# 0xMiden/miden-vm

Hardware: NVIDIA H100
Metric: trace cells/sec proved (higher is better)
Workload: dtype u64

## Files before the change

miden-vm_b200/csrc/kernels.cu:

```cuda
#include "kernels.cuh"
#include "poseidon2.cuh"
#include "poseidon2_fast2.cuh"
#include "ntt2.cuh"
#include "blake3.cuh"
#include "keccak.cuh"
#include "rescue.cuh"
#include <algorithm>
#include <cstdio>

namespace mk {

static unsigned long long g_launches = 0;
unsigned long long launch_count() { return g_launches; }
void count_launch() { ++g_launches; }
void reset_launch_count() { g_launches = 0; }
#define COUNT_LAUNCH() (++g_launches)

void upload_constants() {
    cudaMemcpyToSymbol(p2::D_RC_EXT_INITIAL, p2::P2_RC_EXT_INITIAL, sizeof(u64) * 48);
    cudaMemcpyToSymbol(p2::D_RC_INTERNAL, p2::P2_RC_INTERNAL, sizeof(u64) * 22);
    cudaMemcpyToSymbol(p2::D_RC_EXT_TERMINAL, p2::P2_RC_EXT_TERMINAL, sizeof(u64) * 48);
    cudaMemcpyToSymbol(rsc::D_ARK1, rsc::RESCUE_ARK1, sizeof(u64) * 84);
    cudaMemcpyToSymbol(rsc::D_ARK2, rsc::RESCUE_ARK2, sizeof(u64) * 84);
}

#ifdef MDN_EMULATED
static inline void st_release_sys(u64* p, u64 v) { __atomic_store_n(p, v, __ATOMIC_RELEASE); }
static inline u64 ld_acquire_sys(const u64* p) { return __atomic_load_n(p, __ATOMIC_ACQUIRE); }
static constexpr long long BARRIER_TIMEOUT = 600ll * 1000000000ll;
#else
__device__ __forceinline__ void st_release_sys(u64* p, u64 v) { asm volatile("st.release.sys.global.u64 [%0], %1;" ::"l"(p), "l"(v) : "memory"); }
__device__ __forceinline__ u64 ld_acquire_sys(const u64* p) { u64 v; asm volatile("ld.acquire.sys.global.u64 %0, [%1];" : "=l"(v) : "l"(p) : "memory"); return v; }
static constexpr long long BARRIER_TIMEOUT = 30000000000ll;
#endif
__device__ __forceinline__ void push_u2(const PushDst& d, size_t idx, size_t owner_key, ulonglong2 v) {
    if (d.mode == PUSH_ALL) {
        for (u32 g = 0; g < d.world; g++) reinterpret_cast<ulonglong2*>(d.pp.p[g])[idx] = v;
    } else {
        u32 g = d.mode == PUSH_OWNER ? (u32)(owner_key >> d.owner_shift) : d.rank;
        reinterpret_cast<ulonglong2*>(d.pp.p[g])[idx] = v;
    }
}
struct BarrierArgs { PeerPtrs flags; u32 rank, world; u64 epoch; u32* err; };
__global__ void k_barrier(BarrierArgs a) {
    u32 p = threadIdx.x;
    if (p < a.world) { __threadfence_system(); st_release_sys(a.flags.p[p] + a.rank, a.epoch); }
    __syncthreads();
    if (p < a.world) {
        long long t0 = clock64();
        while (ld_acquire_sys(a.flags.p[a.rank] + p) < a.epoch) {
            if (clock64() - t0 > BARRIER_TIMEOUT) { atomicOr(a.err, 8u); break; }
#ifdef MDN_EMULATED
            emu::cpu_relax();
#endif
        }
    }
}
void launch_barrier(const PeerPtrs& flags, u32 rank, u32 world, u64 epoch, u32* err, cudaStream_t st) {
    BarrierArgs a; a.flags = flags; a.rank = rank; a.world = world; a.epoch = epoch; a.err = err;
    k_barrier<<<1, 32, 0, st>>>(a);
    COUNT_LAUNCH();
}
struct PushArgs { const u64* src; PeerPtrs dst; u32 rank, world; size_t n; };
__global__ void __launch_bounds__(256) k_push(PushArgs a) {
    size_t stride = (size_t)gridDim.x * blockDim.x, i0 = (size_t)blockIdx.x * blockDim.x + threadIdx.x;
    if ((a.n & 1) == 0 && (((size_t)a.src) & 15) == 0) {
        const ulonglong2* s2 = reinterpret_cast<const ulonglong2*>(a.src);
        for (size_t i = i0; i < a.n / 2; i += stride) {
            ulonglong2 v = s2[i];
            for (u32 g = 0; g < a.world; g++) if (g != a.rank) reinterpret_cast<ulonglong2*>(a.dst.p[g])[i] = v;
        }
    } else {
        for (size_t i = i0; i < a.n; i += stride) {
            u64 v = a.src[i];
            for (u32 g = 0; g < a.world; g++) if (g != a.rank) a.dst.p[g][i] = v;
        }
    }
}
void launch_push(const u64* src, const PeerPtrs& dst, u32 rank, u32 world, size_t n, cudaStream_t st) {
    if (!n || world <= 1) return;
    PushArgs a; a.src = src; a.dst = dst; a.rank = rank; a.world = world; a.n = n;
    unsigned blocks = (unsigned)std::min<size_t>((n / 2 + 255) / 256 + 1, 132 * 8);
    k_push<<<blocks, 256, 0, st>>>(a);
    COUNT_LAUNCH();
}

struct TransposeDst { PeerPtrs dst; PeerPtrs bad; u32 world; };
__global__ void k_transpose(const u64* __restrict__ src, TransposeDst d, u32 n_rows, u32 width, size_t col_stride, u32 row0) {
    __shared__ u64 tile[32][33];
    u32 r0 = blockIdx.x * 32, c0 = blockIdx.y * 32;
    bool any_bad = false;
    for (u32 i = threadIdx.y; i < 32; i += 8) {
        u32 r = r0 + i, c = c0 + threadIdx.x;
        if (r < n_rows && c < width) {
            u64 v = src[(size_t)r * width + c];
            any_bad |= (v >= gl::P);
            tile[i][threadIdx.x] = v;
        }
    }
    if (any_bad) for (u32 g = 0; g < d.world; g++) if (d.bad.p[g]) atomicOr(reinterpret_cast<u32*>(d.bad.p[g]), 1u);
    __syncthreads();
    for (u32 i = threadIdx.y; i < 32; i += 8) {
        u32 c = c0 + i, r = r0 + threadIdx.x;
        if (r < n_rows && c < width) {
            u64 v = tile[threadIdx.x][i];
            size_t o = (size_t)c * col_stride + row0 + r;
            for (u32 g = 0; g < d.world; g++) d.dst.p[g][o] = v;
        }
    }
}
void launch_transpose_rm_to_cm(const u64* src, u64* dst, u32 n_rows, u32 width, u32* d_bad_flag, cudaStream_t st) {
    TransposeDst d{}; d.dst.p[0] = dst; d.bad.p[0] = reinterpret_cast<u64*>(d_bad_flag); d.world = 1;
    dim3 grid((n_rows + 31) / 32, (width + 31) / 32), block(32, 8);
    k_transpose<<<grid, block, 0, st>>>(src, d, n_rows, width, (size_t)n_rows, 0u);
    COUNT_LAUNCH();
}
void launch_transpose_slice_push(const u64* src_slice, const PeerPtrs& dst_cm, const PeerPtrs& bad, u32 world, u32 row0, u32 n_rows_slice,
                                 u32 n_rows_total, u32 width, cudaStream_t st) {
    if (!n_rows_slice || !width) return;
    TransposeDst d{}; d.dst = dst_cm; d.bad = bad; d.world = world;
    dim3 grid((n_rows_slice + 31) / 32, (width + 31) / 32), block(32, 8);
    k_transpose<<<grid, block, 0, st>>>(src_slice, d, n_rows_slice, width, (size_t)n_rows_total, row0);
    COUNT_LAUNCH();
}

static constexpr int NTT_THREADS = 256;
static inline unsigned ntt_threads(u32 m, u32 log_cols) {
    u32 g = (m + log_cols >= 3) ? (1u << (m + log_cols - 3)) : 1u;
    if (g < 32) g = 32;
    if (g > 256) g = 256;
    return g;
}

__device__ __forceinline__ u64 w_pow(const u64* __restrict__ hi, const u64* __restrict__ lo, u32 lo_bits, u64 e) {
    return gl::mul(hi[e >> lo_bits], lo[e & ((1ull << lo_bits) - 1)]);
}

#define NTT_BOUNDS __launch_bounds__(NTT_THREADS)
template <int N1C, int N2C>
__global__ void NTT_BOUNDS k_intt_strided(u64* cols, size_t col_stride, NttTables T, u32 log_c) {
    extern __shared__ u64 sm[];
    ntt2::intt_strided_block<N1C, N2C>(blockIdx.x, blockIdx.y, sm, cols, col_stride, T, log_c);
}
template <int N2C>
__global__ void NTT_BOUNDS k_intt_contig(u64* cols, size_t col_stride, NttTables T) {
    extern __shared__ u64 sm[];
    ntt2::intt_contig_block<N2C>(blockIdx.x, blockIdx.y, sm, cols, col_stride, T);
}
template <int N1C, int N2C>
__global__ void NTT_BOUNDS k_fwd_contig(const FwdItem* __restrict__ items, NttTables T, PremulTables Pm) {
    extern __shared__ u64 sm[];
    ntt2::fwd_contig_block<N1C, N2C>(blockIdx.x, blockIdx.y, sm, items, T, Pm);
}
template <int N1C, int N2C>
__global__ void NTT_BOUNDS k_fwd_strided(const FwdItem* __restrict__ items, NttTables T, u32 log_c) {
    extern __shared__ u64 sm[];
    ntt2::fwd_strided_block<N1C, N2C>(blockIdx.x, blockIdx.y, sm, items, T, log_c);
}
#define NTT_SPECIALISED(X) X(8, 8) X(8, 9) X(9, 9) X(9, 10) X(10, 10) X(10, 11) X(11, 11)

template <int N1C, int N2C>
static void launch_intt_t(u64* cols, size_t col_stride, u32 n_cols, const NttTables& T, u32 log_c, cudaStream_t st) {
    u32 N1 = 1u << T.n1, N2 = 1u << T.n2, C = 1u << log_c;
    if (T.n1 > 0) {
        size_t smem = ntt2::smem_words_strided(T.n1, log_c) * sizeof(u64);
        cudaFuncSetAttribute(k_intt_strided<N1C, N2C>, cudaFuncAttributeMaxDynamicSharedMemorySize, (int)smem);
        k_intt_strided<N1C, N2C><<<dim3(N2 / C, n_cols), ntt_threads(T.n1, log_c), smem, st>>>(cols, col_stride, T, log_c);
        COUNT_LAUNCH();
    }
    size_t smem = ntt2::smem_words_contig_inv(T.n2) * sizeof(u64);
    k_intt_contig<N2C><<<dim3(N1, n_cols), ntt_threads(T.n2, 0), smem, st>>>(cols, col_stride, T);
    COUNT_LAUNCH();
}
void launch_intt(u64* cols, size_t col_stride, u32 n_cols, const NttTables& T, cudaStream_t st) {
    u32 log_c = T.n1 >= 12 ? 0 : 12 - T.n1; if (log_c > T.n2) log_c = T.n2;
#define X(a, b) if (T.n1 == a && T.n2 == b) { launch_intt_t<a, b>(cols, col_stride, n_cols, T, log_c, st); return; }
    NTT_SPECIALISED(X)
#undef X
    launch_intt_t<-1, -1>(cols, col_stride, n_cols, T, log_c, st);
}
template <int N1C, int N2C>
static void launch_fwd_t(const FwdItem* d_items, u32 n_items, const NttTables& T, const PremulTables& Pm, u32 log_c, cudaStream_t st) {
    u32 N1 = 1u << T.n1, N2 = 1u << T.n2, C = 1u << log_c;
    size_t smem = ntt2::smem_words_contig_fwd(T.n2) * sizeof(u64);
    k_fwd_contig<N1C, N2C><<<dim3(N1, n_items), ntt_threads(T.n2, 0), smem, st>>>(d_items, T, Pm);
    COUNT_LAUNCH();
    if (T.n1 > 0) {
        size_t smem2 = ntt2::smem_words_strided(T.n1, log_c) * sizeof(u64);
        cudaFuncSetAttribute(k_fwd_strided<N1C, N2C>, cudaFuncAttributeMaxDynamicSharedMemorySize, (int)smem2);
        k_fwd_strided<N1C, N2C><<<dim3(N2 / C, n_items), ntt_threads(T.n1, log_c), smem2, st>>>(d_items, T, log_c);
        COUNT_LAUNCH();
    }
}
void launch_fwd_ntt(const FwdItem* d_items, u32 n_items, const NttTables& T, const PremulTables& Pm, cudaStream_t st) {
    u32 log_c = T.n1 >= 12 ? 0 : 12 - T.n1; if (log_c > T.n2) log_c = T.n2;
#define X(a, b) if (T.n1 == a && T.n2 == b) { launch_fwd_t<a, b>(d_items, n_items, T, Pm, log_c, st); return; }
    NTT_SPECIALISED(X)
#undef X
    launch_fwd_t<-1, -1>(d_items, n_items, T, Pm, log_c, st);
}

static constexpr int HASH_THREADS = 128;
static constexpr int HASH_MIN_BLOCKS = 6;

enum { PERM_P2 = 0, PERM_RPO = 3, PERM_RPX = 4 };
template <int PERM>
__device__ __forceinline__ void alg_permute(u64* s) {
    if constexpr (PERM == PERM_RPO) rsc::rpo_permute(s);
    else if constexpr (PERM == PERM_RPX) rsc::rpx_permute(s);
    else p2f::permute(s);
}
#define ALG_BOUNDS(PERM) __launch_bounds__(HASH_THREADS, (PERM) == PERM_P2 ? HASH_MIN_BLOCKS : 1)
#define ALG_DISPATCH(perm, CALL) do { if ((perm) == PERM_RPO) { CALL(PERM_RPO); } else if ((perm) == PERM_RPX) { CALL(PERM_RPX); } else { CALL(PERM_P2); } } while (0)

template <int PERM>
__global__ void ALG_BOUNDS(PERM) k_leaf_hash(LeafArgs a, u32 log_n, u32 log_b, const u64* __restrict__ prev,
                                                            u32 prev_log_n, u64* __restrict__ states_out,
                                                            PushDst dig, u32 has_dig, u32 t0, u32 nt) {
    size_t L = (size_t)1 << (log_n + log_b);
    size_t idx = (size_t)blockIdx.x * blockDim.x + threadIdx.x;
    if (idx >= ((size_t)nt << log_n)) return;
    u32 t = t0 + (u32)(idx >> log_n);
    u32 r = (u32)(idx & (((size_t)1 << log_n) - 1));
    size_t pos = ((size_t)t << log_n) + r;
    u64 s[12];
    if (prev) {
        size_t Lp = (size_t)1 << (prev_log_n + log_b);
        size_t pp = ((size_t)t << prev_log_n) + (r & ((1u << prev_log_n) - 1));
#pragma unroll
        for (int k = 0; k < 12; k++) s[k] = prev[k * Lp + pp];
    } else {
#pragma unroll
        for (int k = 0; k < 12; k++) s[k] = 0;
    }
    for (int m = 0; m < a.n_mats; m++) {
        const u64* base = a.m[m].base + pos;
        u32 w = a.m[m].width;
        for (u32 c0 = 0; c0 < w; c0 += 8) {
#pragma unroll
            for (u32 k = 0; k < 8; k++) s[k] = (c0 + k < w) ? base[(size_t)(c0 + k) * L] : 0ull;
            alg_permute<PERM>(s);
        }
    }
    if (states_out) {
#pragma unroll
        for (int k = 0; k < 12; k++) states_out[k * L + pos] = glf::canon(s[k]);
    }
    if (has_dig) {
        size_t i = ((size_t)r << log_b) | t;
        push_u2(dig, 2 * i, i, make_ulonglong2(glf::canon(s[0]), glf::canon(s[1])));
        push_u2(dig, 2 * i + 1, i, make_ulonglong2(glf::canon(s[2]), glf::canon(s[3])));
    }
}
template <int PERM>
static void launch_leaf_hash_t(const LeafArgs& a, u32 log_n, u32 log_blowup, const u64* prev_states, u32 prev_log_n,
                               u64* states_out, const PushDst* dig, u32 t0, u32 nt, cudaStream_t st) {
    size_t cnt = (size_t)nt << log_n;
    unsigned blocks = (unsigned)((cnt + HASH_THREADS - 1) / HASH_THREADS);
    PushDst d = dig ? *dig : local_dst(nullptr);
    k_leaf_hash<PERM><<<blocks, HASH_THREADS, 0, st>>>(a, log_n, log_blowup, prev_states, prev_log_n, states_out, d, dig ? 1u : 0u, t0, nt);
    COUNT_LAUNCH();
}
void launch_leaf_hash(const LeafArgs& a, u32 log_n, u32 log_blowup, const u64* prev_states, u32 prev_log_n,
                      u64* states_out, const PushDst* dig, u32 t0, u32 nt, cudaStream_t st, int perm) {
#define X(PM) launch_leaf_hash_t<PM>(a, log_n, log_blowup, prev_states, prev_log_n, states_out, dig, t0, nt, st)
    ALG_DISPATCH(perm, X);
#undef X
}

template <int PERM>
__global__ void ALG_BOUNDS(PERM) k_compress(const u64* __restrict__ ch, u64* __restrict__ par, size_t n) {
    size_t i = (size_t)blockIdx.x * blockDim.x + threadIdx.x;
    if (i >= n) return;
    const ulonglong2* c = reinterpret_cast<const ulonglong2*>(ch + i * 8);
    ulonglong2 a0 = c[0], a1 = c[1], b0 = c[2], b1 = c[3];
    u64 s[12] = {a0.x, a0.y, a1.x, a1.y, b0.x, b0.y, b1.x, b1.y, 0, 0, 0, 0};
    alg_permute<PERM>(s);
    ulonglong2* d = reinterpret_cast<ulonglong2*>(par + i * 4);
    d[0] = make_ulonglong2(glf::canon(s[0]), glf::canon(s[1]));
    d[1] = make_ulonglong2(glf::canon(s[2]), glf::canon(s[3]));
}
template <int PERM>
static void launch_compress_layer_t(const u64* children, u64* parents, size_t n_parents, cudaStream_t st) {
    unsigned blocks = (unsigned)((n_parents + HASH_THREADS - 1) / HASH_THREADS);
    k_compress<PERM><<<blocks, HASH_THREADS, 0, st>>>(children, parents, n_parents);
    COUNT_LAUNCH();
}
void launch_compress_layer(const u64* children, u64* parents, size_t n_parents, cudaStream_t st, int perm) {
#define X(PM) launch_compress_layer_t<PM>(children, parents, n_parents, st)
    ALG_DISPATCH(perm, X);
#undef X
}

template <int PERM>
__global__ void __launch_bounds__(HASH_THREADS) k_fri_leaf(const u64* __restrict__ ev, size_t q, u32 la, PushDst dig, u32 log_b, u32 t0, u32 log_nt) {
    size_t idx = (size_t)blockIdx.x * blockDim.x + threadIdx.x;
    if (idx >= ((q >> log_b) << log_nt)) return;
    size_t i = ((idx >> log_nt) << log_b) | (t0 + (idx & ((1u << log_nt) - 1)));
    const ulonglong2* e = reinterpret_cast<const ulonglong2*>(ev);
    u64 s[12];
#pragma unroll
    for (int k = 0; k < 12; k++) s[k] = 0;
    u32 a = 1u << la;
    for (u32 j0 = 0; j0 < a; j0 += 4) {
#pragma unroll
        for (u32 j = 0; j < 4; j++) {
            if (j0 + j < a) {
                ulonglong2 v = e[i + (size_t)gl::bitrev32(j0 + j, la) * q];
                s[2 * j] = v.x; s[2 * j + 1] = v.y;
            } else { s[2 * j] = 0; s[2 * j + 1] = 0; }
        }
        alg_permute<PERM>(s);
    }
    push_u2(dig, 2 * i, i, make_ulonglong2(glf::canon(s[0]), glf::canon(s[1])));
    push_u2(dig, 2 * i + 1, i, make_ulonglong2(glf::canon(s[2]), glf::canon(s[3])));
}
static inline u32 log2_exact(u32 v) { u32 l = 0; while ((1u << l) < v) l++; return l; }
template <int PERM>
static void launch_fri_leaf_hash_t(const u64* evals, size_t rows, u32 log_arity, const PushDst& digests, u32 log_b, u32 t0, u32 nt, cudaStream_t st) {
    if (rows < ((size_t)1 << log_b)) { log_b = 0; t0 = 0; nt = 1; }
    size_t cnt = (rows >> log_b) * nt;
    unsigned blocks = (unsigned)((cnt + HASH_THREADS - 1) / HASH_THREADS);
    k_fri_leaf<PERM><<<blocks, HASH_THREADS, 0, st>>>(evals, rows, log_arity, digests, log_b, t0, log2_exact(nt));
    COUNT_LAUNCH();
}
void launch_fri_leaf_hash(const u64* evals, size_t rows, u32 log_arity, const PushDst& digests, u32 log_b, u32 t0, u32 nt, cudaStream_t st, int perm) {
#define X(PM) launch_fri_leaf_hash_t<PM>(evals, rows, log_arity, digests, log_b, t0, nt, st)
    ALG_DISPATCH(perm, X);
#undef X
}

__global__ void k_p2_batch(u64* st, size_t n) {
    size_t i = (size_t)blockIdx.x * blockDim.x + threadIdx.x;
    if (i >= n) return;
    u64 s[12];
#pragma unroll
    for (int k = 0; k < 12; k++) s[k] = st[i * 12 + k];
    p2f::permute(s);
#pragma unroll
    for (int k = 0; k < 12; k++) st[i * 12 + k] = glf::canon(s[k]);
}
void launch_poseidon2_batch(u64* states, size_t n, cudaStream_t st) {
    k_p2_batch<<<(unsigned)((n + 127) / 128), 128, 0, st>>>(states, n);
// ... 782 lines not shown
```

miden-vm_b200/csrc/ntt2.cuh:

```cuda
#pragma once
#include "poseidon2_fast2.cuh"
#include "kernels.cuh"
#include "tma.cuh"

namespace ntt2 {
using gl::u64;
using gl::u32;

#if defined(__CUDA_ARCH__) || defined(MDN_EMULATED)
#define NTT2_FOR(i, n) for (u32 i = threadIdx.x; i < (u32)(n); i += blockDim.x)
#define NTT2_SYNC() __syncthreads()
#else
#define NTT2_FOR(i, n) for (u32 i = 0; i < (u32)(n); i++)
#define NTT2_SYNC() ((void)0)
#endif

GL_HD u32 tile_off(u32 idx, u32 cc, u32 log_cols) {
    u32 o = (idx << log_cols) + cc;
    return log_cols ? o : o + (o >> 3);
}
GL_HD u32 tile_words(u32 m, u32 log_cols) {
    u32 n = 1u << (m + log_cols);
    return log_cols ? n : n + (n >> 3) + 1;
}
GL_HD u32 tw_off(u32 m, u32 log_cols) { return (tile_words(m, log_cols) + 1u) & ~1u; }
GL_HD size_t smem_words_contig_fwd(u32 n2) { return (size_t)tw_off(n2, 0) + ((size_t)1 << n2) + 2; }
GL_HD size_t smem_words_contig_inv(u32 n2) { return (size_t)tw_off(n2, 0) + ((size_t)1 << n2) / 2 + 4; }
GL_HD size_t smem_words_strided(u32 n1, u32 log_c) { return (size_t)tw_off(n1, log_c) + ((size_t)1 << n1) / 2 + 4; }

GL_HD void load_chunk(u64* x, const u64* src, u32 n) {
#if defined(__CUDA_ARCH__)
    if (n >= 2 && (((size_t)src) & 15) == 0) {
        const ulonglong2* s2 = reinterpret_cast<const ulonglong2*>(src);
        NTT2_FOR(i, n / 2) { ulonglong2 v = s2[i]; x[tile_off(2 * i, 0, 0)] = v.x; x[tile_off(2 * i + 1, 0, 0)] = v.y; }
        return;
    }
#endif
    NTT2_FOR(i, n) x[tile_off(i, 0, 0)] = src[i];
}
GL_HD void store_chunk_canon(u64* dst, const u64* x, u32 n) {
#if defined(__CUDA_ARCH__)
    if (n >= 2 && (((size_t)dst) & 15) == 0) {
        ulonglong2* d2 = reinterpret_cast<ulonglong2*>(dst);
        NTT2_FOR(i, n / 2) d2[i] = make_ulonglong2(glf::canon_cc(x[tile_off(2 * i, 0, 0)]), glf::canon_cc(x[tile_off(2 * i + 1, 0, 0)]));
        return;
    }
#endif
    NTT2_FOR(i, n) dst[i] = glf::canon_cc(x[tile_off(i, 0, 0)]);
}

struct TableLoad { bool async; };
GL_HD TableLoad table_load(u64* dst, const u64* src, u32 words, u64* bar) {
#if defined(__CUDA_ARCH__)
    const u32 bytes = (words * 8u + 15u) & ~15u;
    if (words >= 64 && ((((size_t)src) | ((size_t)dst)) & 15) == 0) {
        if (threadIdx.x == 0) { tma::mbar_init(bar, 1); }
        __syncthreads();
        if (threadIdx.x == 0) { tma::expect_tx(bar, bytes); tma::bulk_g2s(dst, src, bytes, bar); }
        return TableLoad{true};
    }
#endif
    (void)bar;
    NTT2_FOR(i, words) dst[i] = src[i];
    return TableLoad{false};
}
GL_HD void table_wait(TableLoad t, u64* bar) {
#if defined(__CUDA_ARCH__)
    if (t.async) tma::wait(bar, 0);
#endif
    (void)t; (void)bar;
}

template <bool STAGED>
GL_HD u64 tw_at(const u64* tw, u32 m, u32 s, u32 j) { return STAGED ? tw[((1u << s) - 1u) + j] : tw[j << (m - 1 - s)]; }

template <int LOGR, bool STAGED, bool UNIT0>
GL_HD void dit_group(u64* x, const u64* tw, u32 m, u32 b, u32 log_cols, u32 g) {
    constexpr int R = 1 << LOGR;
    u32 cc = g & ((1u << log_cols) - 1), gg = g >> log_cols;
    u32 lo = gg & ((1u << b) - 1), hi = gg >> b;
    u32 base = (hi << (b + LOGR)) | lo;
    u64 v[R];
#pragma unroll
    for (int k = 0; k < R; k++) v[k] = x[tile_off(base + ((u32)k << b), cc, log_cols)];
#pragma unroll
    for (int st = 0; st < LOGR; st++) {
#pragma unroll
        for (int k = 0; k < R; k++) {
            if (k & (1 << st)) continue;
            const u32 jj = (u32)(k & ((1 << st) - 1));
            u64 c;
            if (UNIT0 && jj == 0) c = glf::canon_cc(v[k + (1 << st)]);
            else c = glf::cmul(v[k + (1 << st)], tw_at<STAGED>(tw, m, b + st, lo + (jj << b)));
            u64 a = v[k];
            v[k] = glf::add_const(a, c);
            v[k + (1 << st)] = glf::csub(a, c);
        }
    }
#pragma unroll
    for (int k = 0; k < R; k++) x[tile_off(base + ((u32)k << b), cc, log_cols)] = v[k];
}
template <int LOGR, bool UNIT0>
GL_HD void dif_group(u64* x, const u64* tw, u32 m, u32 b, u32 log_cols, u32 g) {
    constexpr int R = 1 << LOGR;
    u32 cc = g & ((1u << log_cols) - 1), gg = g >> log_cols;
    u32 lo = gg & ((1u << b) - 1), hi = gg >> b;
    u32 base = (hi << (b + LOGR)) | lo;
    u64 v[R];
#pragma unroll
    for (int k = 0; k < R; k++) v[k] = x[tile_off(base + ((u32)k << b), cc, log_cols)];
#pragma unroll
    for (int st = LOGR - 1; st >= 0; st--) {
#pragma unroll
        for (int k = 0; k < R; k++) {
            if (k & (1 << st)) continue;
            const u32 jj = (u32)(k & ((1 << st) - 1));
            u64 a = v[k], c = glf::canon_cc(v[k + (1 << st)]);
            v[k] = glf::add_const(a, c);
            u64 d = glf::csub(a, c);
            v[k + (1 << st)] = (UNIT0 && jj == 0) ? d : glf::mul(d, tw_at<false>(tw, m, b + st, lo + (jj << b)));
        }
    }
#pragma unroll
    for (int k = 0; k < R; k++) x[tile_off(base + ((u32)k << b), cc, log_cols)] = v[k];
}

template <int LOGR, bool STAGED, bool UNIT0>
GL_HD void dit_round(u64* x, const u64* tw, u32 m, u32 b, u32 log_cols) {
    NTT2_FOR(g, 1u << (m - LOGR + log_cols)) dit_group<LOGR, STAGED, UNIT0>(x, tw, m, b, log_cols, g);
    NTT2_SYNC();
}
template <int LOGR, bool UNIT0>
GL_HD void dif_round(u64* x, const u64* tw, u32 m, u32 b, u32 log_cols) {
    NTT2_FOR(g, 1u << (m - LOGR + log_cols)) dif_group<LOGR, UNIT0>(x, tw, m, b, log_cols, g);
    NTT2_SYNC();
}
template <bool STAGED>
GL_HD void smem_dit(u64* x, const u64* tw, u32 m, u32 log_cols) {
    u32 b = 0;
    while (b < m) {
        u32 left = m - b;
        if (left >= 3 && left != 4) {
            if (b == 0) dit_round<3, STAGED, !STAGED>(x, tw, m, b, log_cols); else dit_round<3, STAGED, false>(x, tw, m, b, log_cols);
            b += 3;
        } else if (left == 4 || left == 2) {
            if (b == 0) dit_round<2, STAGED, !STAGED>(x, tw, m, b, log_cols); else dit_round<2, STAGED, false>(x, tw, m, b, log_cols);
            b += 2;
        } else {
            if (b == 0) dit_round<1, STAGED, !STAGED>(x, tw, m, b, log_cols); else dit_round<1, STAGED, false>(x, tw, m, b, log_cols);
            b += 1;
        }
    }
}
GL_HD void smem_dif(u64* x, const u64* tw, u32 m, u32 log_cols) {
    u32 top = m;
    while (top > 0) {
        if (top >= 3 && top != 4) {
            if (top == 3) dif_round<3, true>(x, tw, m, 0, log_cols); else dif_round<3, false>(x, tw, m, top - 3, log_cols);
            top -= 3;
        } else if (top == 4 || top == 2) {
            if (top == 2) dif_round<2, true>(x, tw, m, 0, log_cols); else dif_round<2, false>(x, tw, m, top - 2, log_cols);
            top -= 2;
        } else {
            dif_round<1, true>(x, tw, m, 0, log_cols);
            top -= 1;
        }
    }
}

template <bool STAGED, int M, int LC, int B = 0>
GL_HD void smem_dit_t(u64* x, const u64* tw) {
    if constexpr (B < M) {
        constexpr int left = M - B;
        constexpr int R = (left >= 3 && left != 4) ? 3 : ((left == 4 || left == 2) ? 2 : 1);
        dit_round<R, STAGED, (B == 0) && !STAGED>(x, tw, (u32)M, (u32)B, (u32)LC);
        smem_dit_t<STAGED, M, LC, B + R>(x, tw);
    }
}
template <int M, int LC, int TOP = M>
GL_HD void smem_dif_t(u64* x, const u64* tw) {
    if constexpr (TOP > 0) {
        constexpr int R = (TOP >= 3 && TOP != 4) ? 3 : ((TOP == 4 || TOP == 2) ? 2 : 1);
        dif_round<R, (TOP - R) == 0>(x, tw, (u32)M, (u32)(TOP - R), (u32)LC);
        smem_dif_t<M, LC, TOP - R>(x, tw);
    }
}

GL_HD u64 w_pow(const u64* hi, const u64* lo, u32 lo_bits, u64 e) {
    return glf::mul(hi[e >> lo_bits], lo[e & ((1ull << lo_bits) - 1)]);
}

template <int N1C = -1, int N2C = -1>
GL_HD void intt_strided_block(u32 bx, u32 by, u64* sm, u64* cols, size_t col_stride, const mk::NttTables& T, u32 log_c_rt) {
    const u32 n1 = N1C >= 0 ? (u32)N1C : T.n1, n2 = N2C >= 0 ? (u32)N2C : T.n2;
    const u32 log_c = N1C >= 0 && N2C >= 0 ? (u32)(N1C >= 12 ? 0 : (12 - N1C < N2C ? 12 - N1C : N2C)) : log_c_rt;
    u32 C = 1u << log_c, N1 = 1u << n1, N2 = 1u << n2;
    u64* x = sm; u64* tw = sm + tw_off(n1, log_c); u64* bar = tw + N1 / 2 + 2;
    u64* col = cols + (size_t)by * col_stride;
    u32 j2_0 = bx * C;
    TableLoad tl = table_load(tw, T.twi_n1, N1 / 2, bar);
    NTT2_FOR(idx, N1 * C) {
        u32 j1 = idx >> log_c, cc = idx & (C - 1);
        x[tile_off(j1, cc, log_c)] = col[(size_t)j1 * N2 + j2_0 + cc];
    }
    table_wait(tl, bar);
    NTT2_SYNC();
    if constexpr (N1C >= 0 && N2C >= 0) smem_dif_t<N1C, (N1C >= 12 ? 0 : (12 - N1C < N2C ? 12 - N1C : N2C))>(x, tw);
    else smem_dif(x, tw, n1, log_c);
    NTT2_FOR(idx, N1 * C) {
        u32 slot = idx >> log_c, cc = idx & (C - 1);
        u32 k1 = gl::bitrev32(slot, n1);
        u32 j2 = j2_0 + cc;
        u64 f = w_pow(T.wi_hi, T.wi_lo, T.lo_bits, (u64)j2 * k1);
        col[(size_t)slot * N2 + j2] = glf::cmul(x[tile_off(slot, cc, log_c)], f);
    }
}
template <int N2C = -1>
GL_HD void intt_contig_block(u32 bx, u32 by, u64* sm, u64* cols, size_t col_stride, const mk::NttTables& T) {
    const u32 n2 = N2C >= 0 ? (u32)N2C : T.n2;
    u32 N2 = 1u << n2;
    u64* x = sm; u64* tw = sm + tw_off(n2, 0); u64* bar = tw + N2 / 2 + 2;
    u64* chunk = cols + (size_t)by * col_stride + (size_t)bx * N2;
    TableLoad tl = table_load(tw, T.twi_n2, N2 / 2, bar);
    load_chunk(x, chunk, N2);
    table_wait(tl, bar);
    NTT2_SYNC();
    if constexpr (N2C >= 0) smem_dif_t<N2C, 0>(x, tw); else smem_dif(x, tw, n2, 0);
    store_chunk_canon(chunk, x, N2);
}
static constexpr u32 FWD_LANES = 128;
template <int N1C = -1, int N2C = -1>
GL_HD void fwd_contig_block(u32 bx, u32 by, u64* sm, const mk::FwdItem* items, const mk::NttTables& T, const mk::PremulTables& Pm) {
    const u32 n1 = N1C >= 0 ? (u32)N1C : T.n1, n2 = N2C >= 0 ? (u32)N2C : T.n2, n = N1C >= 0 && N2C >= 0 ? (u32)(N1C + N2C) : T.n;
    u32 N1 = 1u << n1, N2 = 1u << n2;
    u64* x = sm; u64* tw = sm + tw_off(n2, 0); u64* bar = tw + N2;
    mk::FwdItem it = items[by];
    u32 p_hi = bx;
    u32 j1 = gl::bitrev32(p_hi, n1);
    const u64* src = it.src + (size_t)p_hi * N2;
    u64* dst = it.dst + (size_t)p_hi * N2;
    u64 fb = Pm.tab_b[(size_t)it.base * N1 + j1];
    const u64* tc = Pm.tab_c + (size_t)it.base * N2;
    TableLoad tl = table_load(tw, tc, N2, bar);
    load_chunk(x, src, N2);
    table_wait(tl, bar);
    NTT2_SYNC();
    if constexpr (N2C >= 0) smem_dit_t<true, N2C, 0>(x, tw); else smem_dit<true>(x, tw, n2, 0);
    u32 lanes = N2 < FWD_LANES ? N2 : FWD_LANES;
    NTT2_FOR(l, lanes) {
        u64 f = fb, step = 1;
        if (n1 > 0) {
            u64 mask = ((u64)1 << n) - 1;
            f = glf::mul(fb, w_pow(T.w_hi, T.w_lo, T.lo_bits, ((u64)j1 * l) & mask));
            step = w_pow(T.w_hi, T.w_lo, T.lo_bits, ((u64)j1 * lanes) & mask);
        }
        for (u32 k2 = l; k2 < N2; k2 += lanes) {
            dst[k2] = glf::cmul(x[tile_off(k2, 0, 0)], f);
            if (n1 > 0) f = glf::mul(f, step);
        }
    }
}
template <int N1C = -1, int N2C = -1>
GL_HD void fwd_strided_block(u32 bx, u32 by, u64* sm, const mk::FwdItem* items, const mk::NttTables& T, u32 log_c_rt) {
    const u32 n1 = N1C >= 0 ? (u32)N1C : T.n1, n2 = N2C >= 0 ? (u32)N2C : T.n2;
    const u32 log_c = N1C >= 0 && N2C >= 0 ? (u32)(N1C >= 12 ? 0 : (12 - N1C < N2C ? 12 - N1C : N2C)) : log_c_rt;
    u32 C = 1u << log_c, N1 = 1u << n1, N2 = 1u << n2;
    u64* x = sm; u64* tw = sm + tw_off(n1, log_c); u64* bar = tw + N1 / 2 + 2;
    u64* col = items[by].dst;
    u32 k2_0 = bx * C;
    TableLoad tl = table_load(tw, T.tw_n1, N1 / 2, bar);
    NTT2_FOR(idx, N1 * C) {
        u32 p_hi = idx >> log_c, cc = idx & (C - 1);
        x[tile_off(p_hi, cc, log_c)] = col[(size_t)p_hi * N2 + k2_0 + cc];
    }
    table_wait(tl, bar);
    NTT2_SYNC();
    if constexpr (N1C >= 0 && N2C >= 0) smem_dit_t<false, N1C, (N1C >= 12 ? 0 : (12 - N1C < N2C ? 12 - N1C : N2C))>(x, tw);
    else smem_dit<false>(x, tw, n1, log_c);
    NTT2_FOR(idx, N1 * C) {
        u32 k1 = idx >> log_c, cc = idx & (C - 1);
        col[(size_t)k1 * N2 + k2_0 + cc] = glf::canon_cc(x[tile_off(k1, cc, log_c)]);
    }
}

}
```

Measured before the change: 581.2 million.

## Fuse NTT global load/store into first/last butterfly rounds with radix-16 schedule

For the specialised NTT sizes, the first butterfly round now reads straight from global memory into registers and the last round writes results (with twiddle scaling) straight to global. This drops a separate shared-memory load pass and store pass and their barriers. Rounds now use a fixed radix-16/8 schedule with fewer passes, and thread counts are computed from elements per thread. Shared tiles use a padding of one word per 16 to avoid bank conflicts. The change raises register pressure and the launch thread counts must match the schedule.

```diff
diff --git a/miden-vm_b200/csrc/kernels.cu b/miden-vm_b200/csrc/kernels.cu
--- a/miden-vm_b200/csrc/kernels.cu
+++ b/miden-vm_b200/csrc/kernels.cu
@@ -125,8 +125,8 @@
 }
 
 static constexpr int NTT_THREADS = 256;
-static inline unsigned ntt_threads(u32 m, u32 log_cols) {
-    u32 g = (m + log_cols >= 3) ? (1u << (m + log_cols - 3)) : 1u;
+static inline unsigned ntt_threads(u32 m, u32 log_cols, u32 log_elems) {
+    u32 g = (m + log_cols >= log_elems) ? (1u << (m + log_cols - log_elems)) : 1u;
     if (g < 32) g = 32;
     if (g > 256) g = 256;
     return g;
@@ -162,14 +162,15 @@
 template <int N1C, int N2C>
 static void launch_intt_t(u64* cols, size_t col_stride, u32 n_cols, const NttTables& T, u32 log_c, cudaStream_t st) {
     u32 N1 = 1u << T.n1, N2 = 1u << T.n2, C = 1u << log_c;
+    constexpr u32 LOG_E1 = N1C >= 0 ? ntt2::sched_log_elems(N1C) : 3, LOG_E2 = N2C >= 0 ? ntt2::sched_log_elems(N2C) : 3;
     if (T.n1 > 0) {
         size_t smem = ntt2::smem_words_strided(T.n1, log_c) * sizeof(u64);
         cudaFuncSetAttribute(k_intt_strided<N1C, N2C>, cudaFuncAttributeMaxDynamicSharedMemorySize, (int)smem);
-        k_intt_strided<N1C, N2C><<<dim3(N2 / C, n_cols), ntt_threads(T.n1, log_c), smem, st>>>(cols, col_stride, T, log_c);
+        k_intt_strided<N1C, N2C><<<dim3(N2 / C, n_cols), ntt_threads(T.n1, log_c, LOG_E1), smem, st>>>(cols, col_stride, T, log_c);
         COUNT_LAUNCH();
     }
     size_t smem = ntt2::smem_words_contig_inv(T.n2) * sizeof(u64);
-    k_intt_contig<N2C><<<dim3(N1, n_cols), ntt_threads(T.n2, 0), smem, st>>>(cols, col_stride, T);
+    k_intt_contig<N2C><<<dim3(N1, n_cols), ntt_threads(T.n2, 0, LOG_E2), smem, st>>>(cols, col_stride, T);
     COUNT_LAUNCH();
 }
 void launch_intt(u64* cols, size_t col_stride, u32 n_cols, const NttTables& T, cudaStream_t st) {
@@ -182,13 +183,14 @@
 template <int N1C, int N2C>
 static void launch_fwd_t(const FwdItem* d_items, u32 n_items, const NttTables& T, const PremulTables& Pm, u32 log_c, cudaStream_t st) {
     u32 N1 = 1u << T.n1, N2 = 1u << T.n2, C = 1u << log_c;
+    constexpr u32 LOG_E1 = N1C >= 0 ? ntt2::sched_log_elems(N1C) : 3, LOG_E2 = N2C >= 0 ? ntt2::sched_log_elems(N2C) : 3;
     size_t smem = ntt2::smem_words_contig_fwd(T.n2) * sizeof(u64);
-    k_fwd_contig<N1C, N2C><<<dim3(N1, n_items), ntt_threads(T.n2, 0), smem, st>>>(d_items, T, Pm);
+    k_fwd_contig<N1C, N2C><<<dim3(N1, n_items), ntt_threads(T.n2, 0, LOG_E2), smem, st>>>(d_items, T, Pm);
     COUNT_LAUNCH();
     if (T.n1 > 0) {
         size_t smem2 = ntt2::smem_words_strided(T.n1, log_c) * sizeof(u64);
         cudaFuncSetAttribute(k_fwd_strided<N1C, N2C>, cudaFuncAttributeMaxDynamicSharedMemorySize, (int)smem2);
-        k_fwd_strided<N1C, N2C><<<dim3(N2 / C, n_items), ntt_threads(T.n1, log_c), smem2, st>>>(d_items, T, log_c);
+        k_fwd_strided<N1C, N2C><<<dim3(N2 / C, n_items), ntt_threads(T.n1, log_c, LOG_E1), smem2, st>>>(d_items, T, log_c);
         COUNT_LAUNCH();
     }
 }
diff --git a/miden-vm_b200/csrc/ntt2.cuh b/miden-vm_b200/csrc/ntt2.cuh
--- a/miden-vm_b200/csrc/ntt2.cuh
+++ b/miden-vm_b200/csrc/ntt2.cuh
@@ -21,32 +21,37 @@
 }
 GL_HD u32 tile_words(u32 m, u32 log_cols) {
     u32 n = 1u << (m + log_cols);
-    return log_cols ? n : n + (n >> 3) + 1;
+    return log_cols ? n + (n >> 4) : n + (n >> 3) + 1;
 }
 GL_HD u32 tw_off(u32 m, u32 log_cols) { return (tile_words(m, log_cols) + 1u) & ~1u; }
 GL_HD size_t smem_words_contig_fwd(u32 n2) { return (size_t)tw_off(n2, 0) + ((size_t)1 << n2) + 2; }
 GL_HD size_t smem_words_contig_inv(u32 n2) { return (size_t)tw_off(n2, 0) + ((size_t)1 << n2) / 2 + 4; }
 GL_HD size_t smem_words_strided(u32 n1, u32 log_c) { return (size_t)tw_off(n1, log_c) + ((size_t)1 << n1) / 2 + 4; }
 
+GL_HD u32 pad16(u32 o) { return o + (o >> 4); }
+template <bool P16 = false>
+GL_HD u32 chunk_off(u32 i) { return P16 ? pad16(i) : tile_off(i, 0, 0); }
+template <bool P16 = false>
 GL_HD void load_chunk(u64* x, const u64* src, u32 n) {
 #if defined(__CUDA_ARCH__)
     if (n >= 2 && (((size_t)src) & 15) == 0) {
         const ulonglong2* s2 = reinterpret_cast<const ulonglong2*>(src);
-        NTT2_FOR(i, n / 2) { ulonglong2 v = s2[i]; x[tile_off(2 * i, 0, 0)] = v.x; x[tile_off(2 * i + 1, 0, 0)] = v.y; }
+        NTT2_FOR(i, n / 2) { ulonglong2 v = s2[i]; x[chunk_off<P16>(2 * i)] = v.x; x[chunk_off<P16>(2 * i + 1)] = v.y; }
         return;
     }
 #endif
-    NTT2_FOR(i, n) x[tile_off(i, 0, 0)] = src[i];
-}
+    NTT2_FOR(i, n) x[chunk_off<P16>(i)] = src[i];
+}
+template <bool P16 = false>
 GL_HD void store_chunk_canon(u64* dst, const u64* x, u32 n) {
 #if defined(__CUDA_ARCH__)
     if (n >= 2 && (((size_t)dst) & 15) == 0) {
         ulonglong2* d2 = reinterpret_cast<ulonglong2*>(dst);
-        NTT2_FOR(i, n / 2) d2[i] = make_ulonglong2(glf::canon_cc(x[tile_off(2 * i, 0, 0)]), glf::canon_cc(x[tile_off(2 * i + 1, 0, 0)]));
+        NTT2_FOR(i, n / 2) d2[i] = make_ulonglong2(glf::canon_cc(x[chunk_off<P16>(2 * i)]), glf::canon_cc(x[chunk_off<P16>(2 * i + 1)]));
         return;
     }
 #endif
-    NTT2_FOR(i, n) dst[i] = glf::canon_cc(x[tile_off(i, 0, 0)]);
+    NTT2_FOR(i, n) dst[i] = glf::canon_cc(x[chunk_off<P16>(i)]);
 }
 
 struct TableLoad { bool async; };
@@ -75,14 +80,8 @@
 GL_HD u64 tw_at(const u64* tw, u32 m, u32 s, u32 j) { return STAGED ? tw[((1u << s) - 1u) + j] : tw[j << (m - 1 - s)]; }
 
 template <int LOGR, bool STAGED, bool UNIT0>
-GL_HD void dit_group(u64* x, const u64* tw, u32 m, u32 b, u32 log_cols, u32 g) {
+GL_HD void dit_bfly(u64* v, const u64* tw, u32 m, u32 b, u32 lo) {
     constexpr int R = 1 << LOGR;
-    u32 cc = g & ((1u << log_cols) - 1), gg = g >> log_cols;
-    u32 lo = gg & ((1u << b) - 1), hi = gg >> b;
-    u32 base = (hi << (b + LOGR)) | lo;
-    u64 v[R];
-#pragma unroll
-    for (int k = 0; k < R; k++) v[k] = x[tile_off(base + ((u32)k << b), cc, log_cols)];
 #pragma unroll
     for (int st = 0; st < LOGR; st++) {
 #pragma unroll
@@ -97,8 +96,35 @@
             v[k + (1 << st)] = glf::csub(a, c);
         }
     }
+}
+template <int LOGR, bool STAGED, bool UNIT0>
+GL_HD void dit_group(u64* x, const u64* tw, u32 m, u32 b, u32 log_cols, u32 g) {
+    constexpr int R = 1 << LOGR;
+    u32 cc = g & ((1u << log_cols) - 1), gg = g >> log_cols;
+    u32 lo = gg & ((1u << b) - 1), hi = gg >> b;
+    u32 base = (hi << (b + LOGR)) | lo;
+    u64 v[R];
+#pragma unroll
+    for (int k = 0; k < R; k++) v[k] = x[tile_off(base + ((u32)k << b), cc, log_cols)];
+    dit_bfly<LOGR, STAGED, UNIT0>(v, tw, m, b, lo);
 #pragma unroll
     for (int k = 0; k < R; k++) x[tile_off(base + ((u32)k << b), cc, log_cols)] = v[k];
+}
+template <int LOGR, bool UNIT0>
+GL_HD void dif_bfly(u64* v, const u64* tw, u32 m, u32 b, u32 lo) {
+    constexpr int R = 1 << LOGR;
+#pragma unroll
+    for (int st = LOGR - 1; st >= 0; st--) {
+#pragma unroll
+        for (int k = 0; k < R; k++) {
+            if (k & (1 << st)) continue;
+            const u32 jj = (u32)(k & ((1 << st) - 1));
+            u64 a = v[k], c = glf::canon_cc(v[k + (1 << st)]);
+            v[k] = glf::add_const(a, c);
+            u64 d = glf::csub(a, c);
+            v[k + (1 << st)] = (UNIT0 && jj == 0) ? d : glf::mul(d, tw_at<false>(tw, m, b + st, lo + (jj << b)));
+        }
+    }
 }
 template <int LOGR, bool UNIT0>
 GL_HD void dif_group(u64* x, const u64* tw, u32 m, u32 b, u32 log_cols, u32 g) {
@@ -109,18 +135,7 @@
     u64 v[R];
 #pragma unroll
     for (int k = 0; k < R; k++) v[k] = x[tile_off(base + ((u32)k << b), cc, log_cols)];
-#pragma unroll
-    for (int st = LOGR - 1; st >= 0; st--) {
-#pragma unroll
-        for (int k = 0; k < R; k++) {
-            if (k & (1 << st)) continue;
-            const u32 jj = (u32)(k & ((1 << st) - 1));
-            u64 a = v[k], c = glf::canon_cc(v[k + (1 << st)]);
-            v[k] = glf::add_const(a, c);
-            u64 d = glf::csub(a, c);
-            v[k + (1 << st)] = (UNIT0 && jj == 0) ? d : glf::mul(d, tw_at<false>(tw, m, b + st, lo + (jj << b)));
-        }
-    }
+    dif_bfly<LOGR, UNIT0>(v, tw, m, b, lo);
 #pragma unroll
     for (int k = 0; k < R; k++) x[tile_off(base + ((u32)k << b), cc, log_cols)] = v[k];
 }
@@ -168,51 +183,105 @@
     }
 }
 
-template <bool STAGED, int M, int LC, int B = 0>
-GL_HD void smem_dit_t(u64* x, const u64* tw) {
-    if constexpr (B < M) {
-        constexpr int left = M - B;
-        constexpr int R = (left >= 3 && left != 4) ? 3 : ((left == 4 || left == 2) ? 2 : 1);
-        dit_round<R, STAGED, (B == 0) && !STAGED>(x, tw, (u32)M, (u32)B, (u32)LC);
-        smem_dit_t<STAGED, M, LC, B + R>(x, tw);
-    }
-}
-template <int M, int LC, int TOP = M>
-GL_HD void smem_dif_t(u64* x, const u64* tw) {
-    if constexpr (TOP > 0) {
-        constexpr int R = (TOP >= 3 && TOP != 4) ? 3 : ((TOP == 4 || TOP == 2) ? 2 : 1);
-        dif_round<R, (TOP - R) == 0>(x, tw, (u32)M, (u32)(TOP - R), (u32)LC);
-        smem_dif_t<M, LC, TOP - R>(x, tw);
+GL_HD constexpr int sched_rounds(int m) { return m == 8 ? 2 : 3; }
+GL_HD constexpr int sched_radix(int m, int i) { return m == 9 ? 3 : (i < 2 && (m != 10 || i == 0)) ? 4 : 3; }
+GL_HD constexpr int sched_span(int m, int i) { return i == 0 ? 0 : sched_span(m, i - 1) + sched_radix(m, i - 1); }
+GL_HD constexpr int sched_log_elems(int m) { return m == 9 ? 3 : 4; }
+
+template <int LOGR, int B, int LC>
+GL_HD void tile_get(u64 (&v)[1 << LOGR], const u64* x, u32 base, u32 cc) {
+#pragma unroll
+    for (int k = 0; k < (1 << LOGR); k++) v[k] = x[pad16(((base + ((u32)k << B)) << LC) + cc)];
+}
+template <int LOGR, int B, int LC>
+GL_HD void tile_put(u64* x, const u64 (&v)[1 << LOGR], u32 base, u32 cc) {
+#pragma unroll
+    for (int k = 0; k < (1 << LOGR); k++) x[pad16(((base + ((u32)k << B)) << LC) + cc)] = v[k];
+}
+template <bool STAGED, int M, int LC, int I, class Ld, class St>
+GL_HD void dit_sched(u64* x, const u64* tw, TableLoad tl, u64* bar, const Ld& ld, const St& st) {
+    constexpr int R = sched_radix(M, I), B = sched_span(M, I);
+    constexpr bool FIRST = I == 0, LAST = I + 1 == sched_rounds(M);
+    NTT2_FOR(g, 1u << (M + LC - R)) {
+        const u32 cc = g & ((1u << LC) - 1), gg = g >> LC, lo = gg & ((1u << B) - 1);
+        const u32 base = ((gg >> B) << (B + R)) | lo;
+        u64 v[1 << R];
+        if constexpr (FIRST) { ld(v, base, cc); table_wait(tl, bar); } else tile_get<R, B, LC>(v, x, base, cc);
+        dit_bfly<R, STAGED, B == 0 && !STAGED>(v, tw, (u32)M, (u32)B, lo);
+        if constexpr (LAST) st(v, base, cc); else tile_put<R, B, LC>(x, v, base, cc);
+    }
+    if constexpr (!LAST) {
+        NTT2_SYNC();
+        dit_sched<STAGED, M, LC, I + 1>(x, tw, tl, bar, ld, st);
+    }
+}
+template <int M, int LC, int I, class Ld, class St>
+GL_HD void dif_sched(u64* x, const u64* tw, TableLoad tl, u64* bar, const Ld& ld, const St& st) {
+    constexpr int R = sched_radix(M, I), B = sched_span(M, I);
+    constexpr bool FIRST = I + 1 == sched_rounds(M), LAST = I == 0;
+    NTT2_FOR(g, 1u << (M + LC - R)) {
+        const u32 cc = g & ((1u << LC) - 1), gg = g >> LC, lo = gg & ((1u << B) - 1);
+        const u32 base = ((gg >> B) << (B + R)) | lo;
+        u64 v[1 << R];
+        if constexpr (FIRST) { ld(v, base, cc); table_wait(tl, bar); } else tile_get<R, B, LC>(v, x, base, cc);
+        dif_bfly<R, B == 0>(v, tw, (u32)M, (u32)B, lo);
+        if constexpr (LAST) st(v, base, cc); else tile_put<R, B, LC>(x, v, base, cc);
+    }
+    if constexpr (!LAST) {
+        NTT2_SYNC();
+        dif_sched<M, LC, I - 1>(x, tw, tl, bar, ld, st);
     }
 }
 
 GL_HD u64 w_pow(const u64* hi, const u64* lo, u32 lo_bits, u64 e) {
     return glf::mul(hi[e >> lo_bits], lo[e & ((1ull << lo_bits) - 1)]);
 }
+
+template <int N1C, int N2C> GL_HD constexpr int strided_log_c() { return N1C >= 12 ? 0 : (12 - N1C < N2C ? 12 - N1C : N2C); }
 
 template <int N1C = -1, int N2C = -1>
 GL_HD void intt_strided_block(u32 bx, u32 by, u64* sm, u64* cols, size_t col_stride, const mk::NttTables& T, u32 log_c_rt) {
     const u32 n1 = N1C >= 0 ? (u32)N1C : T.n1, n2 = N2C >= 0 ? (u32)N2C : T.n2;
-    const u32 log_c = N1C >= 0 && N2C >= 0 ? (u32)(N1C >= 12 ? 0 : (12 - N1C < N2C ? 12 - N1C : N2C)) : log_c_rt;
+    const u32 log_c = N1C >= 0 && N2C >= 0 ? (u32)strided_log_c<N1C, N2C>() : log_c_rt;
     u32 C = 1u << log_c, N1 = 1u << n1, N2 = 1u << n2;
     u64* x = sm; u64* tw = sm + tw_off(n1, log_c); u64* bar = tw + N1 / 2 + 2;
     u64* col = cols + (size_t)by * col_stride;
     u32 j2_0 = bx * C;
     TableLoad tl = table_load(tw, T.twi_n1, N1 / 2, bar);
-    NTT2_FOR(idx, N1 * C) {
-        u32 j1 = idx >> log_c, cc = idx & (C - 1);
-        x[tile_off(j1, cc, log_c)] = col[(size_t)j1 * N2 + j2_0 + cc];
-    }
-    table_wait(tl, bar);
-    NTT2_SYNC();
-    if constexpr (N1C >= 0 && N2C >= 0) smem_dif_t<N1C, (N1C >= 12 ? 0 : (12 - N1C < N2C ? 12 - N1C : N2C))>(x, tw);
-    else smem_dif(x, tw, n1, log_c);
-    NTT2_FOR(idx, N1 * C) {
-        u32 slot = idx >> log_c, cc = idx & (C - 1);
-        u32 k1 = gl::bitrev32(slot, n1);
-        u32 j2 = j2_0 + cc;
-        u64 f = w_pow(T.wi_hi, T.wi_lo, T.lo_bits, (u64)j2 * k1);
-        col[(size_t)slot * N2 + j2] = glf::cmul(x[tile_off(slot, cc, log_c)], f);
+    if constexpr (N1C >= 0 && N2C >= 0) {
+        constexpr int LC = strided_log_c<N1C, N2C>(), NR = sched_rounds(N1C);
+        constexpr int RF = sched_radix(N1C, NR - 1), BF = sched_span(N1C, NR - 1), RL = sched_radix(N1C, 0);
+        static_assert(BF + RF == N1C, "the rounds cover the pass");
+        if (!tl.async) NTT2_SYNC();
+        auto ld = [&](u64 (&v)[1 << RF], u32 base, u32 cc) {
+#pragma unroll
+            for (int k = 0; k < (1 << RF); k++) v[k] = col[(size_t)(base + ((u32)k << BF)) * N2 + j2_0 + cc];
+        };
+        auto st = [&](u64 (&v)[1 << RL], u32 base, u32 cc) {
+            const u32 j2 = j2_0 + cc;
+#pragma unroll
+            for (int k = 0; k < (1 << RL); k++) {
+                const u32 slot = base + (u32)k;
+                u64 f = w_pow(T.wi_hi, T.wi_lo, T.lo_bits, (u64)j2 * gl::bitrev32(slot, n1));
+                col[(size_t)slot * N2 + j2] = glf::cmul(v[k], f);
+            }
+        };
+        dif_sched<N1C, LC, NR - 1>(x, tw, tl, bar, ld, st);
+    } else {
+        NTT2_FOR(idx, N1 * C) {
+            u32 j1 = idx >> log_c, cc = idx & (C - 1);
+            x[tile_off(j1, cc, log_c)] = col[(size_t)j1 * N2 + j2_0 + cc];
+        }
+        table_wait(tl, bar);
+        NTT2_SYNC();
+        smem_dif(x, tw, n1, log_c);
+        NTT2_FOR(idx, N1 * C) {
+            u32 slot = idx >> log_c, cc = idx & (C - 1);
+            u32 k1 = gl::bitrev32(slot, n1);
+            u32 j2 = j2_0 + cc;
+            u64 f = w_pow(T.wi_hi, T.wi_lo, T.lo_bits, (u64)j2 * k1);
+            col[(size_t)slot * N2 + j2] = glf::cmul(x[tile_off(slot, cc, log_c)], f);
+        }
     }
 }
 template <int N2C = -1>
@@ -222,11 +291,25 @@
     u64* x = sm; u64* tw = sm + tw_off(n2, 0); u64* bar = tw + N2 / 2 + 2;
     u64* chunk = cols + (size_t)by * col_stride + (size_t)bx * N2;
     TableLoad tl = table_load(tw, T.twi_n2, N2 / 2, bar);
-    load_chunk(x, chunk, N2);
-    table_wait(tl, bar);
-    NTT2_SYNC();
-    if constexpr (N2C >= 0) smem_dif_t<N2C, 0>(x, tw); else smem_dif(x, tw, n2, 0);
-    store_chunk_canon(chunk, x, N2);
+    if constexpr (N2C >= 0) {
+        constexpr int NR = sched_rounds(N2C), RF = sched_radix(N2C, NR - 1), BF = sched_span(N2C, NR - 1), RL = sched_radix(N2C, 0);
+        static_assert(BF + RF == N2C, "the rounds cover the pass");
+        if (!tl.async) NTT2_SYNC();
+        auto ld = [&](u64 (&v)[1 << RF], u32 base, u32) {
+#pragma unroll
+            for (int k = 0; k < (1 << RF); k++) v[k] = chunk[base + ((u32)k << BF)];
+        };
+        auto st = [&](u64 (&v)[1 << RL], u32 base, u32) { tile_put<RL, 0, 0>(x, v, base, 0); };
+        dif_sched<N2C, 0, NR - 1>(x, tw, tl, bar, ld, st);
+        NTT2_SYNC();
+        store_chunk_canon<true>(chunk, x, N2);
+    } else {
+        load_chunk(x, chunk, N2);
+        table_wait(tl, bar);
+        NTT2_SYNC();
+        smem_dif(x, tw, n2, 0);
+        store_chunk_canon(chunk, x, N2);
+    }
 }
 static constexpr u32 FWD_LANES = 128;
 template <int N1C = -1, int N2C = -1>
@@ -242,45 +325,79 @@
     u64 fb = Pm.tab_b[(size_t)it.base * N1 + j1];
     const u64* tc = Pm.tab_c + (size_t)it.base * N2;
     TableLoad tl = table_load(tw, tc, N2, bar);
-    load_chunk(x, src, N2);
-    table_wait(tl, bar);
-    NTT2_SYNC();
-    if constexpr (N2C >= 0) smem_dit_t<true, N2C, 0>(x, tw); else smem_dit<true>(x, tw, n2, 0);
-    u32 lanes = N2 < FWD_LANES ? N2 : FWD_LANES;
-    NTT2_FOR(l, lanes) {
-        u64 f = fb, step = 1;
-        if (n1 > 0) {
-            u64 mask = ((u64)1 << n) - 1;
-            f = glf::mul(fb, w_pow(T.w_hi, T.w_lo, T.lo_bits, ((u64)j1 * l) & mask));
-            step = w_pow(T.w_hi, T.w_lo, T.lo_bits, ((u64)j1 * lanes) & mask);
-        }
-        for (u32 k2 = l; k2 < N2; k2 += lanes) {
-            dst[k2] = glf::cmul(x[tile_off(k2, 0, 0)], f);
-            if (n1 > 0) f = glf::mul(f, step);
+    if constexpr (N1C >= 0 && N2C >= 0) {
+        constexpr int NR = sched_rounds(N2C), RF = sched_radix(N2C, 0), RL = sched_radix(N2C, NR - 1), BL = sched_span(N2C, NR - 1);
+        static_assert(BL + RL == N2C, "the rounds cover the pass");
+        load_chunk<true>(x, src, N2);
+        NTT2_SYNC();
+        const u64 mask = ((u64)1 << n) - 1;
+        const u64 step = w_pow(T.w_hi, T.w_lo, T.lo_bits, ((u64)j1 << BL) & mask);
+        auto ld = [&](u64 (&v)[1 << RF], u32 base, u32) { tile_get<RF, 0, 0>(v, x, base, 0); };
+        auto st = [&](u64 (&v)[1 << RL], u32 base, u32) {
+            u64 f = glf::mul(fb, w_pow(T.w_hi, T.w_lo, T.lo_bits, ((u64)j1 * base) & mask));
+#pragma unroll
+            for (int k = 0; k < (1 << RL); k++) {
+                dst[base + ((u32)k << BL)] = glf::cmul(v[k], f);
+                if (k + 1 < (1 << RL)) f = glf::mul(f, step);
+            }
+        };
+        dit_sched<true, N2C, 0, 0>(x, tw, tl, bar, ld, st);
+    } else {
+        load_chunk(x, src, N2);
+        table_wait(tl, bar);
+        NTT2_SYNC();
+        smem_dit<true>(x, tw, n2, 0);
+        u32 lanes = N2 < FWD_LANES ? N2 : FWD_LANES;
+        NTT2_FOR(l, lanes) {
+            u64 f = fb, step = 1;
+            if (n1 > 0) {
+                u64 mask = ((u64)1 << n) - 1;
+                f = glf::mul(fb, w_pow(T.w_hi, T.w_lo, T.lo_bits, ((u64)j1 * l) & mask));
+                step = w_pow(T.w_hi, T.w_lo, T.lo_bits, ((u64)j1 * lanes) & mask);
+            }
+            for (u32 k2 = l; k2 < N2; k2 += lanes) {
+                dst[k2] = glf::cmul(x[tile_off(k2, 0, 0)], f);
+                if (n1 > 0) f = glf::mul(f, step);
+            }
         }
     }
 }
 template <int N1C = -1, int N2C = -1>
 GL_HD void fwd_strided_block(u32 bx, u32 by, u64* sm, const mk::FwdItem* items, const mk::NttTables& T, u32 log_c_rt) {
     const u32 n1 = N1C >= 0 ? (u32)N1C : T.n1, n2 = N2C >= 0 ? (u32)N2C : T.n2;
-    const u32 log_c = N1C >= 0 && N2C >= 0 ? (u32)(N1C >= 12 ? 0 : (12 - N1C < N2C ? 12 - N1C : N2C)) : log_c_rt;
+    const u32 log_c = N1C >= 0 && N2C >= 0 ? (u32)strided_log_c<N1C, N2C>() : log_c_rt;
     u32 C = 1u << log_c, N1 = 1u << n1, N2 = 1u << n2;
     u64* x = sm; u64* tw = sm + tw_off(n1, log_c); u64* bar = tw + N1 / 2 + 2;
     u64* col = items[by].dst;
     u32 k2_0 = bx * C;
     TableLoad tl = table_load(tw, T.tw_n1, N1 / 2, bar);
-    NTT2_FOR(idx, N1 * C) {
-        u32 p_hi = idx >> log_c, cc = idx & (C - 1);
-        x[tile_off(p_hi, cc, log_c)] = col[(size_t)p_hi * N2 + k2_0 + cc];
-    }
-    table_wait(tl, bar);
-    NTT2_SYNC();
-    if constexpr (N1C >= 0 && N2C >= 0) smem_dit_t<false, N1C, (N1C >= 12 ? 0 : (12 - N1C < N2C ? 12 - N1C : N2C))>(x, tw);
-    else smem_dit<false>(x, tw, n1, log_c);
-    NTT2_FOR(idx, N1 * C) {
-        u32 k1 = idx >> log_c, cc = idx & (C - 1);
-        col[(size_t)k1 * N2 + k2_0 + cc] = glf::canon_cc(x[tile_off(k1, cc, log_c)]);
-    }
-}
-
-}
+    if constexpr (N1C >= 0 && N2C >= 0) {
+        constexpr int LC = strided_log_c<N1C, N2C>(), NR = sched_rounds(N1C), RF = sched_radix(N1C, 0);
+        constexpr int RL = sched_radix(N1C, NR - 1), BL = sched_span(N1C, NR - 1);
+        static_assert(BL + RL == N1C, "the rounds cover the pass");
+        if (!tl.async) NTT2_SYNC();
+        auto ld = [&](u64 (&v)[1 << RF], u32 base, u32 cc) {
+#pragma unroll
+            for (int k = 0; k < (1 << RF); k++) v[k] = col[(size_t)(base + (u32)k) * N2 + k2_0 + cc];
+        };
+        auto st = [&](u64 (&v)[1 << RL], u32 base, u32 cc) {
+#pragma unroll
+            for (int k = 0; k < (1 << RL); k++) col[(size_t)(base + ((u32)k << BL)) * N2 + k2_0 + cc] = glf::canon_cc(v[k]);
+        };
+        dit_sched<false, N1C, LC, 0>(x, tw, tl, bar, ld, st);
+    } else {
+        NTT2_FOR(idx, N1 * C) {
+            u32 p_hi = idx >> log_c, cc = idx & (C - 1);
+            x[tile_off(p_hi, cc, log_c)] = col[(size_t)p_hi * N2 + k2_0 + cc];
+        }
+        table_wait(tl, bar);
+        NTT2_SYNC();
+        smem_dit<false>(x, tw, n1, log_c);
+        NTT2_FOR(idx, N1 * C) {
+            u32 k1 = idx >> log_c, cc = idx & (C - 1);
+            col[(size_t)k1 * N2 + k2_0 + cc] = glf::canon_cc(x[tile_off(k1, cc, log_c)]);
+        }
+    }
+}
+
+}
```

New measurement: 600.2 million, median of 6. 1.03x the previous value.
